# scrubbbbs/cbird

Measured on AMD Instinct MI355X. Metric: Hamming comparisons/sec + images hashed/sec, 1M-image index, 1/2/4/8 MI355X, higher is better.
Workload: dtype u64 hashes as 64 x FP4 signs, f32 accumulate (find, exact) / u8+f32 (hash)

## Files before the change

cbird_amd/csrc/hamm64_mfma.hip:

```cpp
#include <algorithm>
#include <mutex>
#include <vector>

#include "cbh_internal.h"
#include "fp4_sign.h"

namespace cbh {
namespace {

typedef _Float16 h2 __attribute__((ext_vector_type(2)));
typedef unsigned v4u_t __attribute__((ext_vector_type(4)));

constexpr int kThreads = 256;
constexpr int kWaves = 4;
constexpr int kHT = 8;
constexpr int kG = 2;
constexpr int e8m0(int e) { return (int)((uint32_t)(127 + e) * 0x01010101u); }

constexpr uint32_t kNeedlePad = 384;
constexpr uint32_t kNeedleBytes = 80;
struct NeedleScratch {
  uint32_t nq_pad;
  __host__ __device__ constexpr uint32_t words() const { return 0u; }
  __host__ __device__ constexpr uint32_t fold() const { return 2u * nq_pad; }
  __host__ __device__ constexpr uint32_t pre48() const { return 3u * nq_pad; }
  __host__ __device__ constexpr uint32_t pre16() const { return pre48() + nq_pad / 128u * 192u; }
  __host__ __device__ constexpr uint32_t total() const { return pre16() + nq_pad / 128u * 64u; }
};
static_assert(kNeedlePad % 64u == 0 && kNeedlePad % 96u == 0 && kNeedlePad % 128u == 0,
              "whole pairs, triples and quadruples of needle tiles");
static_assert(NeedleScratch{kNeedlePad}.total() * 16u == kNeedlePad * kNeedleBytes &&
                  NeedleScratch{5u * kNeedlePad}.total() * 16u == 5u * kNeedlePad * kNeedleBytes,
              "the regions add up to kNeedleBytes per padded needle");

__global__ __launch_bounds__(256) void k_expand_needles(const uint64_t* __restrict__ q, uint32_t nq,
                                                        uint32_t nq_pad, uint4* __restrict__ qx) {
  const uint32_t i = blockIdx.x * 256u + threadIdx.x;
  const NeedleScratch L{nq_pad};
  if (i >= L.total()) return;
  const uint32_t* w = reinterpret_cast<const uint32_t*>(q);
  if (i < L.fold()) {
    qx[i] = fp4_expand32((i >> 1) < nq ? w[i] : 0u);
  } else if (i < L.pre48()) {
    const uint32_t j = i - L.fold();
    qx[i] = fp4_expand32(j < nq ? w[2u * j] ^ w[2u * j + 1u] : 0u);
  } else if (i < L.pre16()) {
    const uint32_t u = i - L.pre48(), quad = u / 192u, m = (u % 192u) >> 6, c = u & 31u, kb = (u >> 5) & 1u;
    uint2 o[2];
#pragma unroll
    for (uint32_t k = 0; k < 2; ++k) {
      const uint32_t s = 2u * (2u * m + kb) + k, j = quad * 128u + (s / 3u) * 32u + c;
      const uint32_t lo = j < nq ? w[2u * j] : 0u, hi = j < nq ? w[2u * j + 1u] : 0u;
      o[k] = fp4_expand16(pre48_sub(lo, hi, s % 3u), s == 3u || s == 7u || s == 9u ? kFp4Four : kFp4Half);
    }
    qx[i] = make_uint4(o[0].x, o[0].y, o[1].x, o[1].y);
  } else {
    const uint32_t u = i - L.pre16(), c = u & 31u, kb = (u >> 5) & 1u;
    const uint32_t j0 = (u >> 6) * 128u + kb * 64u + c, j1 = j0 + 32u;
    const uint2 lo = fp4_expand16(j0 < nq ? fold16(w[2u * j0], w[2u * j0 + 1u]) : 0u, kFp4Half);
    const uint2 hi = fp4_expand16(j1 < nq ? fold16(w[2u * j1], w[2u * j1 + 1u]) : 0u, kFp4Four);
    qx[i] = make_uint4(lo.x, lo.y, hi.x, hi.y);
  }
}

__device__ __forceinline__ uint32_t as_u32(float f) { return __builtin_bit_cast(uint32_t, f); }
__device__ __forceinline__ void wave_order() {
  asm volatile("" ::: "memory");
  __builtin_amdgcn_wave_barrier();
  asm volatile("" ::: "memory");
}
__device__ __forceinline__ uint32_t wave_rank(uint64_t m, uint32_t base = 0u) {
  return __builtin_amdgcn_mbcnt_hi((uint32_t)(m >> 32), __builtin_amdgcn_mbcnt_lo((uint32_t)m, base));
}
__device__ __forceinline__ uint32_t cd_row(uint32_t g, uint32_t lane) { return (g & 3u) + 8u * (g >> 2) + 4u * (lane >> 5); }

struct HitParams {
  uint32_t thresh, n, nq, keep0;
  const uint64_t* q;
  const uint32_t* ids;
  cbh_record* rec;
  unsigned long long cap;
  unsigned long long* total;
  const uint2* hay;
  const uint2* qmask;
};

constexpr uint32_t kOutCap = 128;
__device__ __forceinline__ void out_flush(uint32_t* s_out, uint32_t& nout, const HitParams& hp) {
  if (nout == 0) return;
  wave_order();
  const uint32_t lane = threadIdx.x & 63u;
  unsigned long long base = 0;
  if (lane == 0) base = atomicAdd(hp.total, (unsigned long long)nout);
  const uint32_t blo = (uint32_t)__builtin_amdgcn_readfirstlane((int)(uint32_t)base);
  const uint32_t bhi = (uint32_t)__builtin_amdgcn_readfirstlane((int)(uint32_t)(base >> 32));
  base = ((unsigned long long)bhi << 32) | blo;
  for (uint32_t k = lane; k < nout; k += 64u) {
    const uint2 r = *reinterpret_cast<const uint2*>(&s_out[2u * k]);
    if (base + k < hp.cap) hp.rec[base + k] = ((cbh_record)r.y << 32) | r.x;
  }
  wave_order();
  nout = 0;
}
__device__ __forceinline__ void out_push(uint32_t* s_out, uint32_t& nout, bool has, uint32_t qidx, uint32_t dist,
                                         uint32_t id, const HitParams& hp) {
  const uint64_t m = __builtin_amdgcn_ballot_w64(has);
  if (m == 0) return;
  const uint32_t c = (uint32_t)__popcll(m);
  if (nout + c > kOutCap) out_flush(s_out, nout, hp);
  if (has) *reinterpret_cast<uint2*>(&s_out[2u * wave_rank(m, nout)]) = make_uint2(id, (qidx << 7) | dist);
  nout += c;
}

__device__ __forceinline__ bool mask_ok(const HitParams& hp, uint32_t row, uint32_t qi, uint64_t nv) {
  if (!hp.qmask) return true;
  const uint2 hv = hp.hay[row], mk = hp.qmask[qi];
  return (((hv.x ^ (uint32_t)nv) & mk.x) | ((hv.y ^ (uint32_t)(nv >> 32)) & mk.y)) == 0;
}
__device__ __forceinline__ void out_match(uint32_t* s_out, uint32_t& nout, bool under, uint32_t row, uint32_t qi,
                                          uint64_t nv, uint32_t dist, const HitParams& hp) {
  bool has = false;
  uint32_t id = 0;
  if (under && row < hp.n && mask_ok(hp, row, qi, nv)) {
    id = hp.ids[row];
    has = id != 0 || hp.keep0;
  }
  out_push(s_out, nout, has, qi, dist, id, hp);
}

template <int N, class Step>
__device__ __forceinline__ void needle_loop(const uint4* base, uint32_t voff, uint32_t nsteps, uint32_t last, Step&& step) {
  const __amdgpu_buffer_rsrc_t rsrc = __builtin_amdgcn_make_buffer_rsrc(const_cast<uint4*>(base), 0, (int)0xffffffffu, 0x27000);
  auto load = [&](uint32_t s, uint4 (&o)[N]) __attribute__((always_inline)) {
#pragma unroll
    for (uint32_t m = 0; m < (uint32_t)N; ++m) {
      const v4u_t v = __builtin_amdgcn_raw_buffer_load_b128(rsrc, (int)voff, (int)(min(s * N + m, last) * 1024u), 0);
      o[m] = make_uint4(v.x, v.y, v.z, v.w);
    }
  };
  uint4 x[N], y[N];
  load(0, x);
#pragma unroll 1
  for (uint32_t s = 0; s < nsteps; s += 2) {
    load(min(s + 1, nsteps - 1), y);
    step(s, x);
    if (s + 1 < nsteps) {
      load(min(s + 2, nsteps - 1), x);
      step(s + 1, y);
    }
  }
}
constexpr uint32_t kNoClamp = 0xffffffffu;

constexpr uint32_t kFlagMaskPre = (1u << 5) | (1u << 11) | (1u << 17) | (1u << 23);
constexpr uint32_t kFieldOnes = 1u + (1u << 6) + (1u << 12) + (1u << 18);

constexpr uint32_t kPendCap = 320;
constexpr uint32_t kOutOff = 2u * kPendCap;
constexpr uint32_t kItemOff = kOutOff + 2u * kOutCap;
constexpr uint32_t kItemCap = 63u + 64u * 8u;
constexpr uint32_t kPreQueue = kItemOff + kItemCap + 1u;
static_assert(kPendCap >= 63u + (kHT / kG) * 64u, "pending list: every lane of every group of a step");
static_assert(kG == 2, "a descriptor names the two reduction chains of a group of 32 registers");

template <int A, int B, int G>
__device__ __forceinline__ uint32_t or_regs(const v16f (&c)[G]) {
  static_assert(B - A >= 3, "range");
  uint32_t o = as_u32(c[A >> 4][A & 15]) | as_u32(c[(A + 1) >> 4][(A + 1) & 15]) | as_u32(c[(A + 2) >> 4][(A + 2) & 15]);
#pragma unroll
  for (int r = A + 3; r < B; r += 2)
    o |= as_u32(c[r >> 4][r & 15]) | (r + 1 < B ? as_u32(c[(r + 1) >> 4][(r + 1) & 15]) : 0u);
  return o;
}

#define CBH_SCALED_MFMA(A, B, C, SCALE_B) __builtin_amdgcn_mfma_scale_f32_32x32x64_f8f6f4(A, B, C, 4, 4, 0, kScaleOne, 0, SCALE_B)

struct Pre32 {
  static constexpr int kTiles = kHT, kOps = 2;
  static constexpr uint32_t operands(NeedleScratch L) { return L.fold(); }
  static __device__ __forceinline__ uint32_t last_op(uint32_t n_pairs, uint32_t p0) { return n_pairs - 1u - p0; }
  static __device__ __forceinline__ v8i hay(uint2 hv, uint32_t) { return fp4_operand(fp4_expand32(hv.x ^ hv.y)); }
  static __device__ __forceinline__ uint32_t bias(uint32_t t) { return 16u + (t - 1u); }
  static __device__ __forceinline__ int scale(int m, uint32_t half) {
    return m == 0 ? (half ? e8m0(5) : e8m0(-1)) : (half ? e8m0(17) : e8m0(11));
  }
  static __device__ __forceinline__ void chain(const v8i (&a)[kTiles], int t0, const v8i (&b)[kOps], const v16f& c0,
                                               const int (&sc)[kOps], v16f (&c)[kG]) {
#pragma unroll
    for (int t = 0; t < kG; ++t) c[t] = CBH_SCALED_MFMA(a[t0 + t], b[0], c0, sc[0]);
#pragma unroll
    for (int t = 0; t < kG; ++t) c[t] = CBH_SCALED_MFMA(a[t0 + t], b[1], c[t], sc[1]);
  }
};

struct Pre48 {
  static constexpr int kTiles = 6, kOps = 3;
  static constexpr uint32_t operands(NeedleScratch L) { return L.pre48(); }
  static __device__ __forceinline__ uint32_t last_op(uint32_t, uint32_t) { return kNoClamp; }
  static __device__ __forceinline__ v8i hay(uint2 hv, uint32_t half) {
    const uint32_t e0 = pre48_sub(hv.x, hv.y, 0), e1 = pre48_sub(hv.x, hv.y, 1), e2 = pre48_sub(hv.x, hv.y, 2);
    const uint2 s0 = fp4_expand16(half ? e2 : e0, kFp4Half);
    const uint2 s1 = fp4_expand16(half ? e0 : e1, half ? kFp4Four : kFp4Half);
    const uint2 s2 = fp4_expand16(half ? e1 : e2, kFp4Half);
    const uint2 s3 = fp4_expand16(half ? e2 : e0, half ? kFp4Half : kFp4Four);
    return v8i{(int)s0.x, (int)s0.y, (int)s1.x, (int)s1.y, (int)s2.x, (int)s2.y, (int)s3.x, (int)s3.y};
  }
  static __device__ __forceinline__ uint32_t bias(uint32_t t) { return 8u + t; }
  static __device__ __forceinline__ int scale(int m, uint32_t half) {
    return m == 0 ? e8m0(1) : m == 1 ? (half ? e8m0(10) : e8m0(7)) : (half ? e8m0(19) : e8m0(13));
  }
  static __device__ __forceinline__ void chain(const v8i (&a)[kTiles], int t0, const v8i (&b)[kOps], const v16f& c0,
                                               const int (&sc)[kOps], v16f (&c)[kG]) {
#pragma unroll
    for (int m = 0; m < kOps; ++m)
#pragma unroll
      for (int t = 0; t < kG; ++t) {
        const v8i& h = a[t0 + t];
        c[t] = CBH_SCALED_MFMA((v8i{h[2 * m], h[2 * m + 1], h[2 * m + 2], h[2 * m + 3], 0, 0, 0, 0}), b[m], m ? c[t] : c0, sc[m]);
      }
  }
};

struct Pre16 {
  static constexpr int kTiles = kHT, kOps = 1;
  static constexpr uint32_t operands(NeedleScratch L) { return L.pre16(); }
  static __device__ __forceinline__ uint32_t last_op(uint32_t, uint32_t) { return kNoClamp; }
  static __device__ __forceinline__ v8i hay(uint2 hv, uint32_t) {
    const uint32_t f = fold16(hv.x, hv.y);
    const uint2 s0 = fp4_expand16(f, kFp4Half), s1 = fp4_expand16(f, kFp4Four);
    return v8i{(int)s0.x, (int)s0.y, (int)s1.x, (int)s1.y, 0, 0, 0, 0};
  }
  static __device__ __forceinline__ uint32_t bias(uint32_t t) { return 24u + (t - 1u); }
  static __device__ __forceinline__ int scale(int, uint32_t half) { return half ? e8m0(13) : e8m0(1); }
  static __device__ __forceinline__ void chain(const v8i (&a)[kTiles], int t0, const v8i (&b)[kOps], const v16f& c0,
                                               const int (&sc)[kOps], v16f (&c)[kG]) {
#pragma unroll
    for (int t = 0; t < kG; ++t) c[t] = CBH_SCALED_MFMA(a[t0 + t], b[0], c0, sc[0]);
  }
};

#define CBH_MFMA_PARAMS                                                                                              \
  const uint2 *__restrict__ hay, const uint32_t *__restrict__ ids, uint32_t n, const uint64_t *__restrict__ q,       \
      const uint4 *__restrict__ qx, uint32_t nq, uint32_t n_pairs, uint32_t pairs_per_chunk, uint32_t thresh,        \
      cbh_record *__restrict__ rec, unsigned long long cap, unsigned long long *__restrict__ total, uint32_t keep0,  \
      const uint2 *__restrict__ qmask, const uint4 *__restrict__ qf
#define CBH_MFMA_ARGS hay, ids, n, q, qx, nq, n_pairs, pairs_per_chunk, thresh, rec, cap, total, keep0, qmask, qf

template <class V>
__device__ __forceinline__ void prefilter_body(CBH_MFMA_PARAMS) {
  constexpr int HT = V::kTiles, G = kG;
  __shared__ __attribute__((aligned(16))) uint32_t s_queue_[kWaves][kPreQueue];
  __shared__ __attribute__((aligned(16))) uint2 s_hay_[kWaves][HT * 32];
  const uint32_t lane = threadIdx.x & 63u;
  const uint32_t wave = (uint32_t)__builtin_amdgcn_readfirstlane((int)(threadIdx.x >> 6));
  const uint32_t r = lane & 31u, half = lane >> 5;
  const uint32_t tile0 = (blockIdx.x * kWaves + wave) * HT;
  if (tile0 * 32u >= n) return;
  uint32_t* s_queue = s_queue_[wave];
  uint2* s_hay = s_hay_[wave];
  uint32_t* s_out = s_queue + kOutOff;
  uint32_t nout = 0;

  v8i a[HT];
#pragma unroll
  for (int t = 0; t < HT; ++t) {
    const uint32_t row = (tile0 + t) * 32u + r;
    const uint2 hv = row < n ? hay[row] : make_uint2(0u, 0u);
    a[t] = V::hay(hv, half);
    if (half == 0) s_hay[t * 32 + r] = hv;
  }
  wave_order();
  v16f c0;
#pragma unroll
  for (int g = 0; g < 16; ++g) c0[g] = 8388608.0f + (float)(V::bias(thresh) * kFieldOnes);
  asm volatile("" : "+v"(c0));
  int scale[V::kOps];
#pragma unroll
  for (int m = 0; m < V::kOps; ++m) {
    scale[m] = V::scale(m, half);
    asm volatile("" : "+v"(scale[m]));
  }

  const uint32_t p0 = blockIdx.y * pairs_per_chunk;
  const uint32_t p1 = min(n_pairs, p0 + pairs_per_chunk);
  const HitParams hp = {thresh, n, nq, keep0, q, ids, rec, cap, total, hay, qmask};

  uint32_t npend = 0;
  uint32_t nitem = 0;
  uint32_t* s_item = s_queue + kItemOff;
  auto work = [&](uint32_t idx, bool live) {
    const uint32_t it = s_item[idx];
    const uint32_t f = it & 3u, ch = (it >> 2) & 1u, L = (it >> 3) & 63u, pp = p0 + 2u * (it >> 11);
    const uint32_t row0 = ((it >> 9) & 3u) * 64u;
    const uint32_t qi = pp * 64u + (L & 31u) + 32u * f;
    const uint64_t nv = live && qi < hp.nq ? hp.q[qi] : 0;
    const uint32_t qlo = (uint32_t)nv, qhi = (uint32_t)(nv >> 32);
    const uint32_t rows = nv == 0 ? 0u : ch ? 0xfffe0000u : 0x0001ffffu;
    const uint2* hq = s_hay + row0 + cd_row(16u * ch, L);
    uint32_t hit = 0;
#pragma unroll 1
    for (uint32_t i = 0; i < 5u; ++i) {
      const uint32_t qd = 4u * ch + i;
      const uint4* h4 = reinterpret_cast<const uint4*>(hq + 8u * min(i, 4u - ch));
      const uint4 x = h4[0], y = h4[1];
      const uint32_t d0 = __popc(x.x ^ qlo) + __popc(x.y ^ qhi), d1 = __popc(x.z ^ qlo) + __popc(x.w ^ qhi);
      const uint32_t d2 = __popc(y.x ^ qlo) + __popc(y.y ^ qhi), d3 = __popc(y.z ^ qlo) + __popc(y.w ^ qhi);
      const uint32_t m4 = (d0 < hp.thresh ? 1u : 0u) | (d1 < hp.thresh ? 2u : 0u) | (d2 < hp.thresh ? 4u : 0u) |
                          (d3 < hp.thresh ? 8u : 0u);
      hit |= qd < 8u ? m4 << (4u * qd) : 0u;
    }
    hit &= rows;
    while (__builtin_amdgcn_ballot_w64(hit != 0) != 0) {
      const uint32_t wr = row0 + cd_row((uint32_t)__builtin_ctz(hit | 0x80000000u), L);
      const uint2 hv = s_hay[wr];
      out_match(s_out, nout, hit != 0, tile0 * 32u + wr, qi, nv, __popc(hv.x ^ qlo) + __popc(hv.y ^ qhi), hp);
      hit &= hit - 1u;
    }
  };
  auto drain = [&](bool all) {
    wave_order();
    const uint32_t keep = all ? 0u : (npend & 63u);
    uint32_t k0 = keep;
    for (;;) {
      if (nitem < 64u && k0 < npend) {
        const uint2 e = *reinterpret_cast<const uint2*>(&s_queue[2u * min(k0 + lane, npend - 1u)]);
        uint32_t cm = 0;
#pragma unroll
        for (uint32_t c = 0; c < 2; ++c) {
          const uint32_t w = e.x >> c;
          cm |= (((w >> 23) & 1u) ? 0xfu : (((w >> 5) & 1u) | (((w >> 11) & 1u) << 1) | (((w >> 17) & 1u) << 2))) << (4u * c);
        }
        if (k0 + lane >= npend) cm = 0;
#pragma unroll
        for (uint32_t b = 0; b < 8; ++b) {
          const bool on = ((cm >> b) & 1u) != 0;
          const uint64_t m = __builtin_amdgcn_ballot_w64(on);
          if (on) s_item[wave_rank(m, nitem)] = (e.y << 3) | b;
          nitem += (uint32_t)__popcll(m);
        }
        k0 += 64u;
        wave_order();
        continue;
      }
      uint32_t idx;
      bool live = true;
      if (nitem >= 64u) {
        nitem -= 64u;
        idx = nitem + lane;
      } else if (all && nitem != 0) {
        idx = min(lane, nitem - 1u);
        live = lane < nitem;
        nitem = 0;
      } else {
        break;
      }
      work(idx, live);
      wave_order();
    }
    npend = keep;
  };

  auto detect = [&](const v16f (&c)[G], const uint32_t group, const uint32_t step) __attribute__((always_inline)) {
    constexpr int R = G * 16;
    constexpr int RA = R / 2 + 1;
    const uint32_t half0 = or_regs<0, RA, G>(c), half1 = or_regs<RA, R, G>(c);
    const uint32_t flags = (half0 | half1) & kFlagMaskPre;
    const uint64_t hm = __builtin_amdgcn_ballot_w64(flags != 0);
    if (hm != 0) {
      static_assert(R == 32, "two chains of 17 and 15 registers");
      uint32_t ln = lane;
      asm volatile("" : "+v"(ln));
      if (flags != 0)
        *reinterpret_cast<uint2*>(&s_queue[2u * wave_rank(hm, npend)]) =
            make_uint2((half0 & kFlagMaskPre) | ((half1 & kFlagMaskPre) << 1), ln | (group << 6) | (step << 8));
      npend += (uint32_t)__popcll(hm);
    }
  };

  needle_loop<V::kOps>(qf + (size_t)(p0 >> 1) * (V::kOps * 64u), lane * 16u, (p1 - p0 + 1u) >> 1, V::last_op(n_pairs, p0),
                       [&](const uint32_t s, const uint4 (&nn)[V::kOps]) __attribute__((always_inline)) {
    v8i b[V::kOps];
#pragma unroll
    for (int m = 0; m < V::kOps; ++m) b[m] = fp4_operand(nn[m]);
#pragma unroll
    for (int t0 = 0; t0 < HT; t0 += G) {
      v16f c[G];
      V::chain(a, t0, b, c0, scale, c);
      detect(c, (uint32_t)(t0 / G), s);
    }
    if (npend >= 64u) drain(false);
  });
  if (npend | nitem) drain(true);
  out_flush(s_out, nout, hp);
}

template <bool PRE>
__global__ void k_hamm64_mfma(CBH_MFMA_PARAMS);
template <>
__global__ __launch_bounds__(kThreads, 4) void k_hamm64_mfma<true>(CBH_MFMA_PARAMS) { prefilter_body<Pre32>(CBH_MFMA_ARGS); }
__global__ __launch_bounds__(kThreads, 3) void k_hamm64_mfma48(CBH_MFMA_PARAMS) { prefilter_body<Pre48>(CBH_MFMA_ARGS); }
__global__ __launch_bounds__(kThreads, 4) void k_hamm64_mfma16(CBH_MFMA_PARAMS) { prefilter_body<Pre16>(CBH_MFMA_ARGS); }

__device__ __forceinline__ void load_hay_words(const uint2* __restrict__ hay, uint32_t n, uint32_t tile0, v8i (&a)[kHT]) {
  const uint32_t r = threadIdx.x & 31u, half = (threadIdx.x >> 5) & 1u;
#pragma unroll
  for (int t = 0; t < kHT; ++t) {
    const uint32_t row = (tile0 + t) * 32u + r;
    const uint2 hv = row < n ? hay[row] : make_uint2(0u, 0u);
    a[t] = fp4_operand(fp4_expand32(half ? hv.y : hv.x));
  }
}

constexpr uint32_t kLoZero2 = 0x4080u, kHiZero2 = 0x4B40u;
__device__ __forceinline__ h2 as_h2(float f) { return __builtin_bit_cast(h2, f); }
__device__ __forceinline__ h2 pkmax3(h2 a, h2 b, h2 c) {
  return __builtin_elementwise_maximum(__builtin_elementwise_maximum(a, b), c);
}
__device__ __forceinline__ void handle_tile2(const v16f& c, uint32_t row0, uint32_t p, uint32_t lo_key, uint32_t hi_key,
                                             const HitParams& hp, uint32_t* s_queue, uint32_t* s_out, uint32_t& nout) {
  const uint32_t lane = threadIdx.x & 63u;
  {
    h2 m0 = {0, 0}, m1 = {0, 0};
#pragma unroll
    for (int g = 0; g < 16; g += 4) {
      m0 = pkmax3(m0, as_h2(c[g]), as_h2(c[g + 1]));
      m1 = pkmax3(m1, as_h2(c[g + 2]), as_h2(c[g + 3]));
    }
    const uint32_t tb = __builtin_bit_cast(uint32_t, __builtin_elementwise_maximum(m0, m1));
    if (__builtin_amdgcn_ballot_w64((tb << 16) >= lo_key || tb >= hi_key) == 0) return;
  }
  uint32_t cnt = 0;
#pragma unroll
  for (int g = 0; g < 16; ++g) {
    const uint32_t bits = as_u32(c[g]);
    const bool fh = bits >= hi_key;
    const bool fl = (bits << 16) >= lo_key;
    if (__builtin_amdgcn_ballot_w64(fh || fl) == 0) continue;
    const uint64_t mh = __builtin_amdgcn_ballot_w64(fh);
    if (fh) s_queue[wave_rank(mh, cnt)] = ((kHiZero2 - (bits >> 16)) << 12) | (1u << 10) | ((uint32_t)g << 6) | lane;
    cnt += (uint32_t)__popcll(mh);
    const uint64_t ml = __builtin_amdgcn_ballot_w64(fl);
    if (fl) s_queue[wave_rank(ml, cnt)] = (((kLoZero2 - (bits & 0xffffu)) >> 1) << 12) | ((uint32_t)g << 6) | lane;
    cnt += (uint32_t)__popcll(ml);
  }
  wave_order();
  for (uint32_t k0 = 0; k0 < cnt; k0 += 64u) {
    const uint32_t k = k0 + lane;
    const uint32_t e = s_queue[min(k, cnt - 1u)];
    const uint32_t src = e & 63u, g = (e >> 6) & 15u, field = (e >> 10) & 1u, d = e >> 12;
    const uint32_t row = row0 + cd_row(g, src);
    const uint32_t qi = p * 64u + field * 32u + (src & 31u);
    bool under = false;
    uint64_t nv = 0;
    if (k < cnt && row < hp.n && qi < hp.nq) {
      nv = hp.q[qi];
      under = nv != 0 && d < hp.thresh;
    }
    out_match(s_out, nout, under, row, qi, nv, d, hp);
  }
  wave_order();
}

template <>
__global__ __launch_bounds__(kThreads, 1) void k_hamm64_mfma<false>(CBH_MFMA_PARAMS) {
  constexpr int HT = kHT, G = kG;
  constexpr uint32_t kQueue = 2048;
  __shared__ uint32_t s_queue_[kWaves][kQueue];
  __shared__ uint32_t s_out_[kWaves][2 * kOutCap];
  const uint32_t lane = threadIdx.x & 63u, wave = threadIdx.x >> 6;
  const uint32_t tile0 = (blockIdx.x * kWaves + wave) * HT;
  if (tile0 * 32u >= n) return;
  uint32_t* s_queue = s_queue_[wave];
  uint32_t* s_out = s_out_[wave];
  uint32_t nout = 0;

  v8i a[HT];
  load_hay_words(hay, n, tile0, a);
  v16f c0;
#pragma unroll
  for (int g = 0; g < 16; ++g) c0[g] = 8388608.0f + 16448.0f + 2097152.0f;
  asm volatile("" : "+v"(c0));
  const uint32_t lo_key = (kLoZero2 - 2u * (thresh - 1u)) << 16, hi_key = (kHiZero2 - (thresh - 1u)) << 16;
  const HitParams hp = {thresh, n, nq, keep0, q, ids, rec, cap, total, hay, qmask};

  const uint32_t p0 = blockIdx.y * pairs_per_chunk;
  const uint32_t p1 = min(n_pairs, p0 + pairs_per_chunk);
  needle_loop<2>(qx + (size_t)p0 * 128u, (2u * (lane & 31u) + (lane >> 5)) * 16u, p1 - p0, kNoClamp,
                 [&](const uint32_t s, const uint4 (&nn)[2]) __attribute__((always_inline)) {
    const v8i bA = fp4_operand(nn[0]), bB = fp4_operand(nn[1]);
#pragma unroll
    for (int t0 = 0; t0 < HT; t0 += G) {
      v16f c[G];
#pragma unroll
      for (int t = 0; t < G; ++t) c[t] = CBH_SCALED_MFMA(a[t0 + t], bA, c0, kScaleOne);
#pragma unroll
      for (int t = 0; t < G; ++t) c[t] = CBH_SCALED_MFMA(a[t0 + t], bB, c[t], e8m0(15));
      h2 m0 = {0, 0}, m1 = {0, 0};
#pragma unroll
      for (int t = 0; t < G; ++t)
#pragma unroll
        for (int g = 0; g < 16; g += 4) {
          m0 = pkmax3(m0, as_h2(c[t][g]), as_h2(c[t][g + 1]));
          m1 = pkmax3(m1, as_h2(c[t][g + 2]), as_h2(c[t][g + 3]));
        }
      const uint32_t mb = __builtin_bit_cast(uint32_t, __builtin_elementwise_maximum(m0, m1));
      if (__builtin_amdgcn_ballot_w64((mb << 16) >= lo_key || mb >= hi_key) != 0) {
#pragma unroll
        for (int t = 0; t < G; ++t)
          handle_tile2(c[t], (tile0 + t0 + t) * 32u, p0 + s, lo_key, hi_key, hp, s_queue, s_out, nout);
      }
    }
  });
  out_flush(s_out, nout, hp);
}
#undef CBH_MFMA_PARAMS
#undef CBH_MFMA_ARGS

constexpr uint32_t kFlagMask3 = (1u << 7) | (1u << 14) | (1u << 21);

__device__ __forceinline__ void handle_tile3(const v16f& c, uint32_t row0, uint32_t p3, const HitParams& hp,
                                             uint32_t* s_queue, uint32_t* s_out, uint32_t& nout) {
  const uint32_t lane = threadIdx.x & 63u;
  uint32_t any = 0;
#pragma unroll
  for (int g = 0; g < 16; ++g) any |= as_u32(c[g]);
  if (__builtin_amdgcn_ballot_w64((any & kFlagMask3) != 0) == 0) return;
  const uint32_t b = hp.thresh - 1u;
#pragma unroll 1
  for (uint32_t f = 0; f < 3; ++f) {
    uint32_t cnt = 0;
#pragma unroll
    for (int g = 0; g < 16; ++g) {
      const uint32_t bits = as_u32(c[g]);
      const bool fl = (bits >> (7u + 7u * f)) & 1u;
      const uint64_t m = __builtin_amdgcn_ballot_w64(fl);
      if (m == 0) continue;
      if (fl)
        s_queue[wave_rank(m, cnt)] = ((64u + b - ((bits >> (1u + 7u * f)) & 0x7fu)) << 12) | (f << 10) | ((uint32_t)g << 6) | lane;
      cnt += (uint32_t)__popcll(m);
    }
    wave_order();
    for (uint32_t k0 = 0; k0 < cnt; k0 += 64u) {
// ... 261 lines not shown
```

cbird_amd/csrc/hamm64_scan.hip:

```cpp
#include <atomic>

#include "cbh_internal.h"

namespace cbh {
namespace {

constexpr int kThreads = 256;
constexpr int kH = 8;
constexpr int kQB = 8;

__device__ __forceinline__ uint32_t min3u(uint32_t a, uint32_t b, uint32_t c) {
  return min(min(a, b), c);
}

__device__ __forceinline__ void emit(cbh_record* __restrict__ rec, unsigned long long cap,
                                     unsigned long long* __restrict__ total, uint32_t qidx,
                                     uint32_t dist, uint32_t id) {
  unsigned long long slot = atomicAdd(total, 1ull);
  if (slot < cap) rec[slot] = ((cbh_record)qidx << 39) | ((cbh_record)dist << 32) | id;
}

template <int H>
__device__ __forceinline__ void exact_block(const uint2 (&h)[H], uint32_t base_idx, uint32_t n,
                                            const uint32_t* __restrict__ ids,
// ... 113 lines not shown
      for (int i = 0; i < QB; ++i) {
        asm volatile("v_mov_b32 %0, %1" : "=v"(ql[i]) : "s"(cur[i].x));
        if (MODE == MODE_FULL) asm volatile("v_mov_b32 %0, %1" : "=v"(qh[i]) : "s"(cur[i].y));
      }
      uint32_t x[QB][H];
      __builtin_amdgcn_sched_barrier(0);
#pragma unroll
      for (int i = 0; i < QB; ++i)
#pragma unroll
        for (int j = 0; j < H; ++j) x[i][j] = h[j].x ^ ql[i];
      __builtin_amdgcn_sched_barrier(0);
      if (MODE == MODE_FULL) {
#pragma unroll
        for (int i = 0; i < QB; ++i)
#pragma unroll
          for (int j = 0; j < H; ++j) x[i][j] = (uint32_t)__popc(x[i][j]);
        uint32_t y[QB][H];
        __builtin_amdgcn_sched_barrier(0);
#pragma unroll
        for (int i = 0; i < QB; ++i)
#pragma unroll
          for (int j = 0; j < H; ++j) y[i][j] = h[j].y ^ qh[i];
        __builtin_amdgcn_sched_barrier(0);
#pragma unroll
        for (int i = 0; i < QB; i += 2)
#pragma unroll
          for (int j = 0; j < H; ++j)
            acc[j] = min3u(acc[j], x[i][j] + (uint32_t)__popc(y[i][j]),
                           x[i + 1][j] + (uint32_t)__popc(y[i + 1][j]));
      } else {
#pragma unroll
        for (int i = 0; i < QB; i += 2)
#pragma unroll
          for (int j = 0; j < H; ++j)
            acc[j] = min3u(acc[j], (uint32_t)__popc(x[i][j]), (uint32_t)__popc(x[i + 1][j]));
      }
      __builtin_amdgcn_sched_barrier(0);
      uint32_t m = acc[0];
#pragma unroll
      for (int j = 1; j + 1 < H; j += 2) m = min3u(m, acc[j], acc[j + 1]);
      if (H % 2 == 0) m = min(m, acc[H - 1]);
      if (m < thresh) refine_block<H, QB>(h, acc, cur, base_idx, n, ids, qb, thresh, rec, cap, total, keep0, qmask);
    }
#pragma unroll
    for (int i = 0; i < QB; ++i) cur[i] = nxt[i];
  }
  if (qb < q1) exact_block<H>(h, base_idx, n, ids, q, qb, q1, thresh, rec, cap, total, keep0, qmask);
}

__global__ __launch_bounds__(256) void k_zero_needle_list(const uint64_t* __restrict__ q, uint32_t nq,
                                                          uint32_t* __restrict__ list ) {
  const uint32_t qi = blockIdx.x * 256u + threadIdx.x;
  if (qi < nq && q[qi] == 0) list[1u + atomicAdd(&list[0], 1u)] = qi;
}

__global__ __launch_bounds__(256) void k_zero_needle_scan(const uint2* __restrict__ hay, const uint32_t* __restrict__ ids,
                                                          uint32_t n, const uint32_t* __restrict__ list, uint32_t thresh,
                                                          cbh_record* __restrict__ rec, unsigned long long cap,
                                                          unsigned long long* __restrict__ total, uint32_t keep0,
                                                          const uint2* __restrict__ qmask) {
  const uint32_t i = blockIdx.x * 256u + threadIdx.x;
  const uint32_t nz = list[0];
  if (i >= n || nz == 0) return;
  const uint2 h = hay[i];
  const uint32_t d = (uint32_t)__popc(h.x) + (uint32_t)__popc(h.y);
  if (d >= thresh) return;
  const uint32_t id = ids[i];
  if (id == 0 && !keep0) return;
  for (uint32_t k = 0; k < nz; ++k) {
    const uint32_t qi = list[1u + k];
    const uint2 mk = qmask ? qmask[qi] : make_uint2(0u, 0u);
    if (((h.x & mk.x) | (h.y & mk.y)) == 0) emit(rec, cap, total, qi, d, id);
  }
}

constexpr unsigned kLoneSlots = 8;
__global__ __launch_bounds__(256) void k_find_one(const uint2* __restrict__ hay, const uint32_t* __restrict__ ids,
                                                  uint32_t n, uint32_t qlo, uint32_t qhi, uint32_t thresh,
                                                  unsigned* __restrict__ d_state, LoneBlock* __restrict__ host,
                                                  unsigned long long seq) {
  const uint32_t base = blockIdx.x * (256u * kLoneSlots) + threadIdx.x;
  bool wrote = false;
#pragma unroll
  for (unsigned k = 0; k < kLoneSlots; ++k) {
    const uint32_t i = base + k * 256u;
    if (i >= n) break;
    const uint2 hv = hay[i];
    const uint32_t d = (uint32_t)__popc(hv.x ^ qlo) + (uint32_t)__popc(hv.y ^ qhi);
    if (d < thresh) {
      const uint32_t id = ids[i];
      if (id != 0) {
        const unsigned slot = atomicAdd(&d_state[0], 1u);
        if (slot < LoneBlock::kRecs) {
          host->recs[slot] = ((cbh_record)d << 32) | id;
          wrote = true;
        }
      }
    }
  }
  if (wrote) __threadfence_system();
  __syncthreads();
  if (threadIdx.x == 0) {
    __threadfence();
    if (atomicAdd(&d_state[1], 1u) == gridDim.x - 1u) {
      __threadfence();
      host->count = atomicExch(&d_state[0], 0u);
      d_state[1] = 0u;
      __threadfence_system();
      __hip_atomic_store(const_cast<unsigned long long*>(&host->done), seq, __ATOMIC_RELEASE, __HIP_MEMORY_SCOPE_SYSTEM);
    }
  }
}

}

int launch_find_one(const uint64_t* d_hashes, const uint32_t* d_ids, size_t n, uint64_t q, int thresh, unsigned* d_state,
                    LoneBlock* h_block, unsigned long long seq, hipStream_t stream) {
  if (n == 0 || n > 0xfffffff0ull || !d_state || !h_block || thresh <= 0) return CBH_E_INVAL;
  const unsigned per_wg = 256u * kLoneSlots;
  hipLaunchKernelGGL(k_find_one, dim3((unsigned)((n + per_wg - 1) / per_wg)), dim3(256), 0, stream,
                     reinterpret_cast<const uint2*>(d_hashes), d_ids, (uint32_t)n, (uint32_t)q, (uint32_t)(q >> 32),
                     (uint32_t)thresh, d_state, h_block, seq);
  CBH_HIP(hipGetLastError());
  return CBH_OK;
}

int wait_find_one(const LoneBlock* h_block, unsigned long long seq, hipStream_t stream) {
  const unsigned long long* flag = const_cast<const unsigned long long*>(&h_block->done);
  for (unsigned spins = 0;; ++spins) {
    if (__atomic_load_n(flag, __ATOMIC_ACQUIRE) == seq) return CBH_OK;
    if ((spins & 0xfffu) == 0xfffu) {
      const hipError_t q = hipStreamQuery(stream);
      if (q == hipSuccess) {
        return __atomic_load_n(flag, __ATOMIC_ACQUIRE) == seq ? CBH_OK : CBH_E_HIP;
      }
      if (q != hipErrorNotReady) {
        set_last_error("k_find_one", q);
        return CBH_E_HIP;
      }
    }
#if defined(__x86_64__)
    __builtin_ia32_pause();
#endif
  }
}

namespace {

constexpr int kPreMax = 7;
constexpr size_t kMfmaMinNq = 256;
constexpr size_t kMfmaMinN = 4096;
constexpr int kPreStatic = 6;
constexpr double kTrueWeight = 8.0;
constexpr double kSlopePre = 1.3e4, kBaseFull = 15.75, kTrueFull = 2.7e5, kTruePre = 0.7e5;
constexpr double kBasePre = 8.55, kBase48 = 14.0, kSlope48 = 2.8e4, kTrue48 = 1.0e5, kPre48Margin = 0.9;
constexpr double kBase16 = 5.85, kPre16Margin = 0.9;
constexpr uint64_t kProbeMinPairs = 1ull << 31;

int g_scan_mfma = 1;
int g_pre_max_thresh = -1;
int g_pre_rate_max_e9 = 300000;
int g_pre48 = -1;
int g_pre16 = -1;
std::atomic<uint64_t> g_variant_mask[4];
std::atomic<uint64_t> g_n_probe{0};
std::atomic<long long> g_last_rate_e9{-1};
std::atomic<long long> g_last_true_e9{-1};
std::atomic<long long> g_last_rate48_e9{-1};
std::atomic<long long> g_last_rate16_e9{-1};

enum class Join { None, IfCheaper, Forced };
enum class Kernel { PopcEq, PopcPre, PopcFull, Mfma };
struct Route {
  Join join;
  Kernel kernel;
  double scan_ms;
};

Route route(size_t n, size_t nq, int thresh, bool masked) {
  Route r;
  const double pairs = (double)n * (double)nq;
  const double pre_ms = pairs * (thresh <= 5 ? 8.7e-12 : thresh == 6 ? 9.7e-12 : thresh == 7 ? 12.1e-12 : 15.8e-12);
  r.scan_ms = thresh == 1 ? pairs * 6.1e-12 : pre_ms;
  const bool joinable = thresh <= kJoinMaxThresh && !masked && n < 0xfffffff0ull;
  r.join = !joinable ? Join::None : g_scan_mfma == 4 ? Join::Forced
           : g_scan_mfma == 3 && pre_ms >= 1.0 ? Join::IfCheaper : Join::None;
  const bool mfma = thresh <= 65 && (g_scan_mfma == 2 || g_scan_mfma == 4 ||
                                     (g_scan_mfma != 0 && nq >= kMfmaMinNq && n >= kMfmaMinN));
  r.kernel = mfma ? Kernel::Mfma : thresh == 1 ? Kernel::PopcEq : thresh <= kPreMax ? Kernel::PopcPre : Kernel::PopcFull;
  return r;
}

void note_variant(int thresh, ScanVariant v) {
  for (int i = 1; i < 4; ++i)
    if (i == (int)v) g_variant_mask[i] |= 1ull << thresh; else g_variant_mask[i] &= ~(1ull << thresh);
}

int launch_popc(Kernel kernel, const uint64_t* d_hashes, const uint32_t* d_ids, size_t n, const uint64_t* d_q, size_t nq,
                int thresh, cbh_record* d_rec, size_t cap, unsigned long long* d_total, hipStream_t stream,
                const ScanOpts& o) {
  const uint32_t tile = kThreads * kH;
  const uint32_t tiles = (uint32_t)((n + tile - 1) / tile);
  const uint32_t q_chunk = scan_chunk(tiles, nq, 16384, 1024, kQB);
  dim3 grid(tiles, (uint32_t)((nq + q_chunk - 1) / q_chunk)), block(kThreads);
  const uint2* hay = reinterpret_cast<const uint2*>(d_hashes);
#define CBH_SCAN(MODE)                                                                                                  \
  hipLaunchKernelGGL((k_hamm64_scan<kH, kQB, MODE>), grid, block, 0, stream, hay, d_ids, (uint32_t)n, d_q, (uint32_t)nq, \
                     q_chunk, (uint32_t)thresh, d_rec, (unsigned long long)cap, d_total, (uint32_t)o.keep_id0,            \
                     reinterpret_cast<const uint2*>(o.d_qmask))
  if (kernel == Kernel::PopcEq) CBH_SCAN(MODE_EQ);
  else if (kernel == Kernel::PopcPre) CBH_SCAN(MODE_PRE);
  else CBH_SCAN(MODE_FULL);
#undef CBH_SCAN
  CBH_HIP(hipGetLastError());
  return CBH_OK;
}

}

bool scan_takes_mfma(size_t n, size_t nq, int thresh) {
  return thresh >= 1 && route(n, nq, thresh, false).kernel == Kernel::Mfma;
}

bool scan_routes_to_join(size_t n, size_t nq, int thresh, bool masked) {
  return thresh >= 1 && n >= 1 && nq >= 1 && route(n, nq, thresh, masked).join != Join::None;
}

ScanVariant scan_pick_pre(const uint64_t* d_hashes, size_t n, size_t n_total, const uint64_t* d_q, size_t nq, int thresh,
                          hipStream_t stream) {
  using V = ScanVariant;
  if (g_pre16 == 1 && thresh <= max_thresh(V::Pre16)) return V::Pre16;
  if (g_pre48 == 1 && thresh <= max_thresh(V::Pre48)) return V::Pre48;
  if (thresh > max_thresh(V::Pre32)) return V::Full;
  if (g_pre_max_thresh >= 0) return thresh <= g_pre_max_thresh ? V::Pre32 : V::Full;
  if (thresh > kProbeMaxThresh) return V::Full;
  double r_cand = 0, r_true = 0, r48 = 0, r16 = 0;
  if ((uint64_t)n_total * (uint64_t)nq < kProbeMinPairs ||
      !probe_fold_rates(d_hashes, n, d_q, nq, thresh, stream, &r_cand, &r_true, &r48, &r16))
    return thresh <= kPreStatic ? V::Pre32 : V::Full;
  g_last_rate_e9 = (long long)(r_cand * 1e9);
  g_last_true_e9 = (long long)(r_true * 1e9);
  g_last_rate48_e9 = (long long)(r48 * 1e9);
  g_last_rate16_e9 = (long long)(r16 * 1e9);
  g_n_probe++;
  const double d_pre = kSlopePre * (r_cand - kTrueWeight * r_true - (double)g_pre_rate_max_e9 * 1e-9);
  const bool pre = d_pre <= 0;
  const double t_pre = kBasePre + kSlopePre * r_cand + kTruePre * r_true, t_full = kBaseFull + kTrueFull * r_true;
  if (g_pre16 != 0 && pre && thresh <= max_thresh(V::Pre16) &&
      kBase16 + kSlopePre * r16 + kTruePre * r_true < kPre16Margin * t_pre)
    return V::Pre16;
  if (g_pre48 != 0) {
    const double t_48 = kBase48 + kSlope48 * r48 + kTrue48 * r_true;
    if (pre ? t_48 < kPre48Margin * t_pre : t_48 < t_full) return V::Pre48;
  }
  return pre ? V::Pre32 : V::Full;
}

namespace {

int launch_zero_needles(const uint64_t* d_hashes, const uint32_t* d_ids, size_t n, const uint64_t* d_q, size_t nq,
                        int thresh, cbh_record* d_rec, size_t cap, unsigned long long* d_total, hipStream_t stream,
                        const ScanOpts& o) {
  Scratch scratch(stream);
  uint32_t* list = nullptr;
  CBH_HIP(scratch.get(&list, (nq + 1) * sizeof(uint32_t)));
  CBH_HIP(hipMemsetAsync(list, 0, sizeof(uint32_t), stream));
  hipLaunchKernelGGL(k_zero_needle_list, dim3((unsigned)((nq + 255) / 256)), dim3(256), 0, stream, d_q, (uint32_t)nq, list);
  hipLaunchKernelGGL(k_zero_needle_scan, dim3((unsigned)((n + 255) / 256)), dim3(256), 0, stream,
                     reinterpret_cast<const uint2*>(d_hashes), d_ids, (uint32_t)n, list, (uint32_t)thresh, d_rec,
                     (unsigned long long)cap, d_total, (uint32_t)o.keep_id0, reinterpret_cast<const uint2*>(o.d_qmask));
  CBH_HIP(hipGetLastError());
  return CBH_OK;
}

int scan_nonzero_needles(const uint64_t* d_hashes, const uint32_t* d_ids, size_t n, const uint64_t* d_q, size_t nq,
                         int thresh, cbh_record* d_rec, size_t cap, unsigned long long* d_total, hipStream_t stream,
                         const ScanOpts& o);

}

int launch_hamm64_scan(const uint64_t* d_hashes, const uint32_t* d_ids, size_t n, const uint64_t* d_q, size_t nq,
                       int thresh, cbh_record* d_rec, size_t cap, unsigned long long* d_total, hipStream_t stream,
                       const ScanOpts& o) {
  if (n == 0 || nq == 0 || thresh <= 0) return CBH_OK;
  if (n > 0xfffffff0ull || nq > CBH_MAX_QUERIES_PER_CALL) return CBH_E_INVAL;
  const int rc = scan_nonzero_needles(d_hashes, d_ids, n, d_q, nq, thresh, d_rec, cap, d_total, stream, o);
  if (rc || !o.zero_needles) return rc;
  return launch_zero_needles(d_hashes, d_ids, n, d_q, nq, thresh, d_rec, cap, d_total, stream, o);
}

namespace {

int scan_nonzero_needles(const uint64_t* d_hashes, const uint32_t* d_ids, size_t n, const uint64_t* d_q, size_t nq,
                         int thresh, cbh_record* d_rec, size_t cap, unsigned long long* d_total, hipStream_t stream,
                         const ScanOpts& o) {
  const Route r = route(n, nq, thresh, o.d_qmask != nullptr);
  if (r.join != Join::None) {
    const bool force = r.join == Join::Forced;
    const int rc = launch_hamm64_join(d_hashes, d_ids, n, d_q, nq, thresh, d_rec, cap, d_total, stream, o, force, r.scan_ms);
    if (rc == CBH_OK || force || (rc != CBH_E_UNSUPPORTED && rc != CBH_E_NOMEM)) return rc;
    if (rc == CBH_E_NOMEM) cbh_clear_error();
  }
  if (r.kernel != Kernel::Mfma) return launch_popc(r.kernel, d_hashes, d_ids, n, d_q, nq, thresh, d_rec, cap, d_total, stream, o);
  const ScanVariant v = o.pre != ScanVariant::Auto ? o.pre : scan_pick_pre(d_hashes, n, n, d_q, nq, thresh, stream);
  if (thresh < 64) note_variant(thresh, v);
  return launch_hamm64_scan_mfma(d_hashes, d_ids, n, d_q, nq, thresh, d_rec, cap, d_total, stream, v, o);
}

}

int set_scan_mfma(int mode) {
  if (mode < 0 || mode > 4) return CBH_E_INVAL;
  g_scan_mfma = mode;
  return CBH_OK;
}
int get_scan_mfma() { return g_scan_mfma; }
void set_scan_pre_max(int t) {
  if (t >= -1 && t <= max_thresh(ScanVariant::Pre32)) g_pre_max_thresh = t;
}
void set_scan_pre_rate(int e9) {
  if (e9 >= 0) g_pre_rate_max_e9 = e9;
}
void set_scan_pre48(int v) {
  if (v >= -1 && v <= 1) g_pre48 = v;
}
long long get_scan_pre_mask() { return (long long)(g_variant_mask[(int)ScanVariant::Pre32] | g_variant_mask[(int)ScanVariant::Pre16]); }
int set_scan_pre16(int v) {
  if (v < -1 || v > 1) return CBH_E_INVAL;
  g_pre16 = v;
  return CBH_OK;
}
long long get_scan_pre48_mask() { return (long long)g_variant_mask[(int)ScanVariant::Pre48].load(); }
long long get_scan_pre16_mask() { return (long long)g_variant_mask[(int)ScanVariant::Pre16].load(); }
long long get_scan_probes() { return (long long)g_n_probe.load(); }
long long get_scan_probe_rate_e9() { return g_last_rate_e9.load(); }
// ... 6 lines not shown
```

Baseline: 78030 billion.

## Batch MFMA prefilter detection per step with struct-of-arrays pending descriptors

The prefilter kernel now ORs the reduction chains of all tile groups into per-lane words and issues a single ballot and queue write per needle step, instead of one per group. Pending descriptors move to a struct-of-arrays layout holding every group's words plus the lane and step id. The drain uses a prefix-sum scatter and takes only as many descriptors as fit in the item buffer. The pending capacity shrinks so LDS fits four workgroups per CU, and the routing cost constants are retuned. The aim is fewer ballots and divergent branches in the hot loop, at the cost of more LDS traffic per flagged lane and a more complex drain.

```diff
diff --git a/cbird_amd/csrc/hamm64_mfma.hip b/cbird_amd/csrc/hamm64_mfma.hip
--- a/cbird_amd/csrc/hamm64_mfma.hip
+++ b/cbird_amd/csrc/hamm64_mfma.hip
@@ -155,13 +155,17 @@
 constexpr uint32_t kFlagMaskPre = (1u << 5) | (1u << 11) | (1u << 17) | (1u << 23);
 constexpr uint32_t kFieldOnes = 1u + (1u << 6) + (1u << 12) + (1u << 18);
 
-constexpr uint32_t kPendCap = 320;
-constexpr uint32_t kOutOff = 2u * kPendCap;
+constexpr uint32_t kGroupsMax = kHT / kG;
+constexpr uint32_t kDescWords = 2u * kGroupsMax + 1u;
+constexpr uint32_t kPendCap = 128;
+constexpr uint32_t kOutOff = kDescWords * kPendCap;
 constexpr uint32_t kItemOff = kOutOff + 2u * kOutCap;
 constexpr uint32_t kItemCap = 63u + 64u * 8u;
 constexpr uint32_t kPreQueue = kItemOff + kItemCap + 1u;
-static_assert(kPendCap >= 63u + (kHT / kG) * 64u, "pending list: every lane of every group of a step");
+static_assert(kPendCap >= 63u + 64u, "pending list: the kept remainder and every lane of a step");
 static_assert(kG == 2, "a descriptor names the two reduction chains of a group of 32 registers");
+static_assert(kItemCap >= 63u + 8u * kGroupsMax, "a pass always takes at least one descriptor");
+static_assert((kPreQueue + kHT * 32u * 2u) * 4u * kWaves <= 40960u, "four workgroups per CU: 40 KB of LDS each");
 
 template <int A, int B, int G>
 __device__ __forceinline__ uint32_t or_regs(const v16f (&c)[G]) {
@@ -249,6 +253,8 @@
 template <class V>
 __device__ __forceinline__ void prefilter_body(CBH_MFMA_PARAMS) {
   constexpr int HT = V::kTiles, G = kG;
+  constexpr int NG = HT / G;
+  static_assert(HT % G == 0 && (uint32_t)NG <= kGroupsMax, "a descriptor holds two words per group");
   __shared__ __attribute__((aligned(16))) uint32_t s_queue_[kWaves][kPreQueue];
   __shared__ __attribute__((aligned(16))) uint2 s_hay_[kWaves][HT * 32];
   const uint32_t lane = threadIdx.x & 63u;
@@ -323,22 +329,33 @@
     uint32_t k0 = keep;
     for (;;) {
       if (nitem < 64u && k0 < npend) {
-        const uint2 e = *reinterpret_cast<const uint2*>(&s_queue[2u * min(k0 + lane, npend - 1u)]);
+        const uint32_t avail = npend - k0;
+        const uint32_t* d = s_queue + min(k0 + lane, npend - 1u);
+        const uint32_t id = d[2u * NG * kPendCap];
         uint32_t cm = 0;
 #pragma unroll
-        for (uint32_t c = 0; c < 2; ++c) {
-          const uint32_t w = e.x >> c;
+        for (uint32_t c = 0; c < 2u * NG; ++c) {
+          const uint32_t w = d[c * kPendCap];
           cm |= (((w >> 23) & 1u) ? 0xfu : (((w >> 5) & 1u) | (((w >> 11) & 1u) << 1) | (((w >> 17) & 1u) << 2))) << (4u * c);
         }
-        if (k0 + lane >= npend) cm = 0;
-#pragma unroll
-        for (uint32_t b = 0; b < 8; ++b) {
-          const bool on = ((cm >> b) & 1u) != 0;
-          const uint64_t m = __builtin_amdgcn_ballot_w64(on);
-          if (on) s_item[wave_rank(m, nitem)] = (e.y << 3) | b;
-          nitem += (uint32_t)__popcll(m);
+        if (lane >= avail) cm = 0;
+        const uint32_t cnt = (uint32_t)__popc(cm);
+        uint32_t off = 0;
+#pragma unroll
+        for (uint32_t b = 0; b < 6; ++b) off += wave_rank(__builtin_amdgcn_ballot_w64(((cnt >> b) & 1u) != 0)) << b;
+        const uint32_t ntake = (uint32_t)__popcll(__builtin_amdgcn_ballot_w64(lane < avail && nitem + off + cnt <= kItemCap));
+        if (lane >= ntake) cm = 0;
+        const uint32_t added = (uint32_t)__builtin_amdgcn_readlane((int)(off + cnt), (int)(ntake - 1u));
+        uint32_t* w = s_item + nitem + off;
+        while (__builtin_amdgcn_ballot_w64(cm != 0) != 0) {
+          if (cm != 0) {
+            const uint32_t b = (uint32_t)__builtin_ctz(cm);
+            *w++ = ((id | ((b >> 3) << 6)) << 3) | (b & 7u);
+            cm &= cm - 1u;
+          }
         }
-        k0 += 64u;
+        nitem += added;
+        k0 += ntake;
         wave_order();
         continue;
       }
@@ -360,19 +377,28 @@
     npend = keep;
   };
 
-  auto detect = [&](const v16f (&c)[G], const uint32_t group, const uint32_t step) __attribute__((always_inline)) {
+  auto reduce = [&](const v16f (&c)[G], const int group, uint32_t (&hw)[2 * NG]) __attribute__((always_inline)) {
     constexpr int R = G * 16;
     constexpr int RA = R / 2 + 1;
-    const uint32_t half0 = or_regs<0, RA, G>(c), half1 = or_regs<RA, R, G>(c);
-    const uint32_t flags = (half0 | half1) & kFlagMaskPre;
-    const uint64_t hm = __builtin_amdgcn_ballot_w64(flags != 0);
+    static_assert(R == 32, "two chains of 17 and 15 registers");
+    hw[2 * group] = or_regs<0, RA, G>(c);
+    hw[2 * group + 1] = or_regs<RA, R, G>(c);
+  };
+  auto detect = [&](const uint32_t (&hw)[2 * NG], const uint32_t step) __attribute__((always_inline)) {
+    uint32_t any = hw[0];
+#pragma unroll
+    for (int i = 1; i < 2 * NG; ++i) any |= hw[i];
+    const bool flagged = (any & kFlagMaskPre) != 0;
+    const uint64_t hm = __builtin_amdgcn_ballot_w64(flagged);
     if (hm != 0) {
-      static_assert(R == 32, "two chains of 17 and 15 registers");
       uint32_t ln = lane;
       asm volatile("" : "+v"(ln));
-      if (flags != 0)
-        *reinterpret_cast<uint2*>(&s_queue[2u * wave_rank(hm, npend)]) =
-            make_uint2((half0 & kFlagMaskPre) | ((half1 & kFlagMaskPre) << 1), ln | (group << 6) | (step << 8));
+      if (flagged) {
+        uint32_t* d = s_queue + wave_rank(hm, npend);
+#pragma unroll
+        for (int i = 0; i < 2 * NG; ++i) d[(uint32_t)i * kPendCap] = hw[i];
+        d[2u * NG * kPendCap] = ln | (step << 8);
+      }
       npend += (uint32_t)__popcll(hm);
     }
   };
@@ -382,12 +408,15 @@
     v8i b[V::kOps];
 #pragma unroll
     for (int m = 0; m < V::kOps; ++m) b[m] = fp4_operand(nn[m]);
+    uint32_t hw[2 * NG];
 #pragma unroll
     for (int t0 = 0; t0 < HT; t0 += G) {
       v16f c[G];
       V::chain(a, t0, b, c0, scale, c);
-      detect(c, (uint32_t)(t0 / G), s);
-    }
+      reduce(c, t0 / G, hw);
+      __builtin_amdgcn_sched_barrier(0);
+    }
+    detect(hw, s);
     if (npend >= 64u) drain(false);
   });
   if (npend | nitem) drain(true);
diff --git a/cbird_amd/csrc/hamm64_scan.hip b/cbird_amd/csrc/hamm64_scan.hip
--- a/cbird_amd/csrc/hamm64_scan.hip
+++ b/cbird_amd/csrc/hamm64_scan.hip
@@ -289,7 +289,7 @@
 constexpr size_t kMfmaMinN = 4096;
 constexpr int kPreStatic = 6;
 constexpr double kTrueWeight = 8.0;
-constexpr double kSlopePre = 1.3e4, kBaseFull = 15.75, kTrueFull = 2.7e5, kTruePre = 0.7e5;
+constexpr double kSlopePre = 1.2e4, kBaseFull = 15.75, kTrueFull = 2.7e5, kTruePre = 0.7e5;
 constexpr double kBasePre = 8.55, kBase48 = 14.0, kSlope48 = 2.8e4, kTrue48 = 1.0e5, kPre48Margin = 0.9;
 constexpr double kBase16 = 5.85, kPre16Margin = 0.9;
 constexpr uint64_t kProbeMinPairs = 1ull << 31;
@@ -317,7 +317,7 @@
 Route route(size_t n, size_t nq, int thresh, bool masked) {
   Route r;
   const double pairs = (double)n * (double)nq;
-  const double pre_ms = pairs * (thresh <= 5 ? 8.7e-12 : thresh == 6 ? 9.7e-12 : thresh == 7 ? 12.1e-12 : 15.8e-12);
+  const double pre_ms = pairs * (thresh <= 5 ? 8.7e-12 : thresh == 6 ? 9.6e-12 : thresh == 7 ? 11.8e-12 : 15.8e-12);
   r.scan_ms = thresh == 1 ? pairs * 6.1e-12 : pre_ms;
   const bool joinable = thresh <= kJoinMaxThresh && !masked && n < 0xfffffff0ull;
   r.join = !joinable ? Join::None : g_scan_mfma == 4 ? Join::Forced
```

Measured after the change: 78710 billion, median of 6. No clear change (+0.9%).
